# snf4j/snf4j

Measured on AMD Instinct MI355X. Metric: WebSocket frame decode GiB/s device-resident at 1/2/4/8 MI355X; % HBM peak, higher is better.
Workload: dtype u8; 1 GPU; 1048576 x 4096 B masked TEXT frames per GPU, 1024 sessions per GPU, unmask + UTF-8 validation, server-side decode (FrameDecoder+FrameUtf8Validator); frames_per_gpu=1048576, payload_bytes=4096, wire_bytes_per_gpu=4303355904, sessions_per_gpu=1024, parallelism=sessions sharded over 1 GPU(s), one process per GPU, no data-path collective

## Files before the change

snf4j_amd/csrc/api.hip:

```cpp
#include <stdarg.h>
#include <stdio.h>
#include <stdlib.h>
#include <string.h>

#include <algorithm>
#include <atomic>
#include <string>
#include <vector>

#include "wsgpu_internal.h"

using namespace ws;

namespace {

std::atomic<uint64_t> g_ctx_allocs{0};

const char* const kKernelNames[K_COUNT] = {"k_parse",   "k_scan",     "k_link",     "k_piecesN",
                                           "k_final",    "k_enc_len",  "k_enc_scan",
                                           "k_enc_piecesN", "k_enc_final", "k_enc_desc", "k_agg_plan", "k_agg_gather", "k_inflate", "k_hs_accept", "k_infl_tok", "k_infl_fast", "k_hs_validate",
                                           "k_defl_plan", "k_defl_prep", "k_defl_match", "k_defl_parse", "k_defl_final", "k_defl_serial",
                                           "k_defl_trees", "k_defl_emit", "k_defl_hist", "k_defl_match_lds", "k_defl_links"};

struct DevBuf {
// ... 16 lines not shown
    p = nullptr;
    n = 0;
  }
};

struct EventPair {
  int kid;
  hipEvent_t a, b;
};

struct HostSlot {
  DevBuf wire, off, sf, state, payload, desc, result;
  hipEvent_t ev_in = nullptr, ev_k = nullptr, ev_state = nullptr, ev_out = nullptr;
  bool used = false;
};

}

struct wsg_ctx {
  int device = 0;
  hipStream_t stream = nullptr;
  bool own_stream = false;
  std::string err;
  DevBuf rec, vflag, slink, edge, blk_sum, blk_max, chunk, sess_err, total, pieces;
  DevBuf esess, elast_close, epieces, epidx;
  DevBuf a_code, a_last, a_pl, a_cl, a_blk, a_sess_err, a_pieces;
  DevBuf v_desc;
  DevBuf i_tok, i_lit, i_stat, i_tab, i_tabcnt, i_fast, i_ord;
  DevBuf i_split;
  DevBuf i_tok2, i_lit2;
  DevBuf d_flags, d_fout, d_fsym, d_ff, d_fs, d_sums, d_S, d_link, d_res, d_tres, d_strips, d_ftail, d_chunks, d_sym, d_tw, d_ssym,
      d_blocks;
  int defl_serial = 0;
  int64_t stage_fail = 0;
  int defl_lds = 1;
  int infl_tokens = 1;
  uint32_t infl_lanes = 262144;
  uint32_t infl_tabs = 32768;
  int infl_fast = 1;
  int infl_lds = 1;
  int infl_order = 1;
  int infl_split = 0;
  int fused_scan = 1;
  int agg_units = 2;
  uint32_t agg_grid = 65536;
  uint32_t agg_fold = 0xFFFFFFFFu;
  uint64_t tok_frames = 0, tok_payload_len = 0;
// ... 118 lines not shown
  wsg_ctx* c = new wsg_ctx();
  c->device = device;
  if (stream) {
    c->stream = (hipStream_t)stream;
  } else {
    if (hipStreamCreateWithFlags(&c->stream, hipStreamNonBlocking) != hipSuccess) {
      delete c;
      return WSG_API_EHIP;
    }
    c->own_stream = true;
  }
  *out = c;
  return WSG_API_OK;
}

int wsg_close(wsg_ctx* c) {
  if (!c) return WSG_API_EINVAL;
  (void)hipSetDevice(c->device);
  if (c->s_in) (void)hipStreamSynchronize(c->s_in);
  (void)hipStreamSynchronize(c->stream);
  if (c->s_out) (void)hipStreamSynchronize(c->s_out);
  drain_timing(c);
  for (auto e : c->free_events) (void)hipEventDestroy(e);
  DevBuf* bufs[] = {&c->rec,     &c->vflag, &c->chunk,    &c->edge,     &c->blk_sum,  &c->blk_max,   &c->sess_err,
                    &c->total,   &c->pieces, &c->slink, &c->esess,   &c->elast_close, &c->epieces, &c->epidx, &c->h_wire, &c->h_off,    &c->h_sf,
                    &c->h_state, &c->h_payload, &c->h_desc, &c->h_result, &c->h_frames, &c->h_closed,
                    &c->h_wire_off};
  for (DevBuf* b : bufs) b->release();
  DevBuf* abufs[] = {&c->a_code, &c->a_last, &c->a_pl, &c->a_cl,
                     &c->a_blk,  &c->a_sess_err, &c->a_pieces, &c->v_desc, &c->i_tok, &c->i_lit,
                     &c->i_stat, &c->i_tab, &c->i_tabcnt, &c->i_fast, &c->i_ord, &c->i_split,
                     &c->i_tok2, &c->i_lit2};
  for (DevBuf* b : abufs) b->release();
  for (HostSlot& hs : c->slot) {
    DevBuf* sb[] = {&hs.wire, &hs.off, &hs.sf, &hs.state, &hs.payload, &hs.desc, &hs.result};
    for (DevBuf* b : sb) b->release();
    hipEvent_t evs[] = {hs.ev_in, hs.ev_k, hs.ev_state, hs.ev_out};
    for (hipEvent_t e : evs)
      if (e) (void)hipEventDestroy(e);
  }
  if (c->s_in) (void)hipStreamDestroy(c->s_in);
  if (c->s_out) (void)hipStreamDestroy(c->s_out);
  if (c->own_stream) (void)hipStreamDestroy(c->stream);
  delete c;
  return WSG_API_OK;
}

// ... 71 lines not shown
  for (int i = 0; i < K_COUNT && i < max_kernels; ++i) {
    if (out_ms) out_ms[i] = c->ms[i];
    if (out_count) out_count[i] = c->count[i];
  }
  return K_COUNT;
}

int wsg_reset_timing(wsg_ctx* c) {
  if (!c) return WSG_API_EINVAL;
  drain_timing(c);
  memset(c->ms, 0, sizeof c->ms);
  memset(c->count, 0, sizeof c->count);
  return WSG_API_OK;
}

static int ensure_decode_ws(wsg_ctx* c, uint64_t n_frames, uint32_t n_sessions, uint64_t wire_len) {
  const uint64_t F = n_frames ? n_frames : 1;
  const uint64_t nblk = (F + DBLOCK - 1) / DBLOCK;
  HIP_TRY(c, c->pieces.ensure((piece_bound(wire_len, F) + 8) * sizeof(PieceDesc)));
  HIP_TRY(c, c->rec.ensure(F * sizeof(FrameRec)));
  HIP_TRY(c, c->vflag.ensure(F));
  HIP_TRY(c, c->slink.ensure(3 * (uint64_t)(n_sessions ? n_sessions : 1) * sizeof(int32_t)));
  HIP_TRY(c, c->edge.ensure(2 * F * sizeof(uint32_t)));
  HIP_TRY(c, c->blk_sum.ensure(nblk * sizeof(uint64_t)));
  HIP_TRY(c, c->blk_max.ensure(4 * ((nblk + 3) & ~3ull) * sizeof(int32_t)));
  HIP_TRY(c, c->chunk.ensure((nblk / SCAN_CHUNK + 1) * (sizeof(uint64_t) + 4 * sizeof(int32_t))));
  HIP_TRY(c, c->sess_err.ensure((uint64_t)(n_sessions ? n_sessions : 1) * sizeof(uint64_t), 0xff, c->stream));
  HIP_TRY(c, c->total.ensure(sizeof(uint64_t)));
  return WSG_API_OK;
}

static int ensure_encode_ws(wsg_ctx* c, uint64_t n_frames) {
  const uint64_t F = n_frames ? n_frames : 1;
  const uint64_t nblk = (F + BLOCK - 1) / BLOCK;
  HIP_TRY(c, c->esess.ensure(F * sizeof(uint32_t)));
  HIP_TRY(c, c->elast_close.ensure(F * sizeof(int32_t)));
  HIP_TRY(c, c->blk_sum.ensure(nblk * sizeof(uint64_t)));
  HIP_TRY(c, c->blk_max.ensure(3 * nblk * sizeof(int32_t)));
  return WSG_API_OK;
}

static constexpr uint64_t INFL_RESIDENT_LANES = 65536;
static bool infl_pairs(const wsg_ctx* c, uint64_t n_frames) {
  return c->infl_lds && (c->infl_split == 2 || (c->infl_split == 1 && 2 * n_frames <= INFL_RESIDENT_LANES));
}
static uint64_t infl_lane_count(const wsg_ctx* c, uint64_t n_frames) {
// ... 87 lines not shown
    return set_err(c, WSG_API_ERANGE, "payload_cap below wsg_decode_payload_bound()");
  HIP_TRY(c, hipSetDevice(c->device));
  int rc = ensure_decode_ws(c, n_frames, n_sessions, wire_len);
  if (rc) return rc;
  DecodeArgs a;
  a.wire = wire;
  a.wire_len = wire_len;
  a.frame_off = frame_off;
  a.n_frames = n_frames;
  a.session_first = session_first;
  a.n_sessions = n_sessions;
  a.client_mode = cfg->client_mode != 0;
  a.allow_ext = cfg->allow_extensions != 0;
  a.validate = cfg->validate_utf8 != 0;
  a.max_payload = cfg->max_payload_len;
  a.state = state;
  a.payload_out = payload_out;
  a.desc = desc_out;
  a.result = result_out;
  a.rec = (FrameRec*)c->rec.p;
  a.vflag = (uint8_t*)c->vflag.p;
  a.slink = (int32_t*)c->slink.p;
  a.edge = (uint32_t*)c->edge.p;
  a.blk_sum = (uint64_t*)c->blk_sum.p;
  a.blk_max = (int32_t*)c->blk_max.p;
  a.chunk_sum = (uint64_t*)c->chunk.p;
  a.chunk_max = (int32_t*)(a.chunk_sum + (n_frames + DBLOCK - 1) / DBLOCK / SCAN_CHUNK + 1);
  a.sess_err = (uint64_t*)c->sess_err.p;
  a.total = (uint64_t*)c->total.p;
  a.pieces = (PieceDesc*)c->pieces.p;
  a.nblk = (uint32_t)((n_frames + DBLOCK - 1) / DBLOCK);
  a.n_pieces = piece_bound(wire_len, n_frames);
  a.validator_only = 0;
  a.in_desc = nullptr;
  a.sparse = (cfg->flags & WSG_CFG_SPARSE) != 0;
  a.fused_scan = a.nblk <= FUSED_SCAN_MAX_BLOCKS && c->fused_scan;
  if (n_frames) {
    timed(c, K_PARSE, [&] { launch_parse(a, c->stream); });
    if (!a.fused_scan) timed(c, K_SCAN, [&] { launch_scan(a, c->stream); });
    timed(c, K_LINK, [&] { launch_link(a, c->stream); });
    timed(c, K_UNMASK, [&] { launch_pieces(a, c->stream, piece_bound(wire_len, n_frames)); });
  }
  timed(c, K_FINAL, [&] { launch_final(a, c->stream); });
  HIP_TRY(c, hipGetLastError());
  return WSG_API_OK;
}
// ... 8 lines not shown
  HIP_TRY(c, hipSetDevice(c->device));
  int rc = ensure_decode_ws(c, n_frames, n_sessions, payload_len);
  if (rc) return rc;
  HIP_TRY(c, c->v_desc.ensure((n_frames + 1) * sizeof(wsg_frame_desc)));
  DecodeArgs a;
  a.wire = payload;
  a.wire_len = payload_len;
  a.frame_off = nullptr;
  a.n_frames = n_frames;
  a.session_first = session_first;
  a.n_sessions = n_sessions;
  a.client_mode = 0;
  a.allow_ext = 1;
  a.validate = 1;
  a.max_payload = INT64_MAX;
  a.state = state;
  a.payload_out = nullptr;
  a.desc = (wsg_frame_desc*)c->v_desc.p;
  a.result = result_out;
  a.rec = (FrameRec*)c->rec.p;
  a.vflag = (uint8_t*)c->vflag.p;
  a.slink = (int32_t*)c->slink.p;
  a.edge = (uint32_t*)c->edge.p;
  a.blk_sum = (uint64_t*)c->blk_sum.p;
  a.blk_max = (int32_t*)c->blk_max.p;
  a.chunk_sum = (uint64_t*)c->chunk.p;
  a.chunk_max = (int32_t*)(a.chunk_sum + (n_frames + DBLOCK - 1) / DBLOCK / SCAN_CHUNK + 1);
  a.sess_err = (uint64_t*)c->sess_err.p;
  a.total = (uint64_t*)c->total.p;
  a.pieces = (PieceDesc*)c->pieces.p;
  a.nblk = (uint32_t)((n_frames + DBLOCK - 1) / DBLOCK);
  a.n_pieces = piece_bound(payload_len, n_frames);
  a.validator_only = 1;
  a.in_desc = desc;
  a.sparse = 0;
  a.fused_scan = a.nblk <= FUSED_SCAN_MAX_BLOCKS && c->fused_scan;
  if (n_frames) {
    timed(c, K_PARSE, [&] { launch_vparse(a, c->stream); });
    if (!a.fused_scan) timed(c, K_SCAN, [&] { launch_scan(a, c->stream); });
    timed(c, K_LINK, [&] { launch_link(a, c->stream); });
    timed(c, K_UNMASK, [&] { launch_vpieces(a, c->stream, a.n_pieces); });
  }
  timed(c, K_FINAL, [&] { launch_final(a, c->stream); });
  HIP_TRY(c, hipGetLastError());
  return WSG_API_OK;
}
// ... 878 lines not shown
```

snf4j_amd/csrc/decode.hip:

```cpp
#include "wsgpu_internal.h"
#include "wsgpu_scan.h"

namespace ws {

__device__ bool utf8_valid_run(const uint8_t* wire, uint64_t off, uint32_t n, uint32_t mask, uint32_t phase0) {
  uint32_t p1 = 0, p2 = 0, p3 = 0;
  for (uint32_t i = 0; i < n; ++i) {
    uint32_t b = wire[off + i] ^ ((mask >> (8 * ((phase0 + i) & 3))) & 0xffu);
    if (utf8_err_byte(p3, p2, p1, b)) return false;
    p3 = p2; p2 = p1; p1 = b;
  }
  return !utf8_incomplete(p3, p2, p1);
}

struct DAgg {
  uint64_t sum;
  int32_t m0, m1, m2;
  uint32_t c3;
};
constexpr DAgg DAGG_ID = {0ull, -1, -1, -1, 0u};
constexpr uint32_t C3_RESET = 1u << 26;
constexpr uint32_t C3_PENDING = 1u << 27;

__device__ __forceinline__ uint32_t carry_op(uint32_t x, uint32_t y) {
  if (y & C3_RESET) return y;
  const uint32_t nx = (x >> 24) & 3u, ny = (y >> 24) & 3u;
  const uint32_t n = nx + ny < 3u ? nx + ny : 3u;
  return ((x & 0xffffffu) >> (8 * ny)) | (y & 0xffffffu) | (n << 24) | (x & (C3_RESET | C3_PENDING));
}
__device__ __forceinline__ DAgg agg_op(const DAgg& x, const DAgg& y) {
  DAgg r;
  r.sum = x.sum + y.sum;
  r.m0 = x.m0 > y.m0 ? x.m0 : y.m0;
  r.m1 = x.m1 > y.m1 ? x.m1 : y.m1;
  r.m2 = x.m2 > y.m2 ? x.m2 : y.m2;
  r.c3 = carry_op(x.c3, y.c3);
  return r;
}
template <int CTRL, int RM>
__device__ __forceinline__ DAgg agg_dpp(const DAgg& v) {
  DAgg t;
  t.sum = dpp_u64<CTRL, RM>(v.sum, 0ull);
  t.m0 = (int32_t)dpp_u32<CTRL, RM>((uint32_t)v.m0, 0xffffffffu);
  t.m1 = (int32_t)dpp_u32<CTRL, RM>((uint32_t)v.m1, 0xffffffffu);
  t.m2 = (int32_t)dpp_u32<CTRL, RM>((uint32_t)v.m2, 0xffffffffu);
  t.c3 = dpp_u32<CTRL, RM>(v.c3, 0u);
  return t;
}

__device__ __forceinline__ uint32_t tail_c3(const wsg_session_state& st) {
  const uint32_t n = st.tail_len < 3 ? st.tail_len : 3u;
  const uint32_t t = (uint32_t)st.tail[0] | ((uint32_t)st.tail[1] << 8) | ((uint32_t)st.tail[2] << 16);
  return C3_RESET | (n << 24) | ((t << (24 - 8 * n)) & 0xffffffu);
}

__device__ __forceinline__ uint32_t resolve_c3(uint32_t c, const wsg_session_state& st) {
  return (c & C3_PENDING) ? carry_op(tail_c3(st), c & ~(C3_RESET | C3_PENDING)) : c;
}

__device__ __forceinline__ DAgg frame_agg(uint64_t k, const FrameRec& r, uint32_t l3, bool sess_first) {
  DAgg v;
// ... 172 lines not shown
}

__global__ __launch_bounds__(DBLOCK) void k_parse(DecodeArgs a) {
  const uint64_t k = (uint64_t)blockIdx.x * DBLOCK + threadIdx.x;
  DAgg v = DAGG_ID;
  if (k < a.n_frames) {
    const uint64_t o = a.frame_off[k], e = a.sparse ? a.wire_len : a.frame_off[k + 1];
    uint32_t d[6];
    const uint64_t a4 = o & ~3ull;
    if (a4 + 24 <= a.wire_len) {
      const uint32_t* p = (const uint32_t*)(a.wire + a4);
#pragma unroll
      for (int j = 0; j < 6; ++j) d[j] = p[j];
    } else {
#pragma unroll
      for (int j = 0; j < 6; ++j) d[j] = 0u;
#pragma unroll
      for (uint32_t b = 0; b < 24u; ++b)
        if (a4 + b < a.wire_len) d[b >> 2] |= (uint32_t)a.wire[a4 + b] << (8 * (b & 3));
    }
    v = parse_one(a, k, o, e, d, wave_session(a, k));
  }
  DAgg tot;
  block_excl_scan_t(v, &tot, DAGG_ID);
  if (threadIdx.x == 0) store_blk(a, blockIdx.x, tot);
}

__device__ __forceinline__ uint32_t plain_byte(const DecodeArgs& a, uint64_t i) { return i < a.wire_len ? a.wire[i] : 0u; }
__device__ __forceinline__ uint32_t plain_word(const DecodeArgs& a, uint64_t i) {
  const uint64_t q = i & ~3ull;
  if (q + 8 <= a.wire_len) {
    const uint32_t lo = *(const uint32_t*)(a.wire + q), hi = *(const uint32_t*)(a.wire + q + 4);
    return alignbyte(hi, lo, (uint32_t)(i & 3u));
  }
  return plain_byte(a, i) | (plain_byte(a, i + 1) << 8) | (plain_byte(a, i + 2) << 16) | (plain_byte(a, i + 3) << 24);
}

__global__ __launch_bounds__(DBLOCK) void k_vparse(DecodeArgs a) {
  const uint64_t k = (uint64_t)blockIdx.x * DBLOCK + threadIdx.x;
  VAgg v = VAGG_ID;
  if (k < a.n_frames) {
    const uint32_t s = wave_session(a, k);
    const wsg_frame_desc d = a.in_desc[k];
    const uint32_t op = d.opcode & 15u, fin = (d.flags >> 7) & 1u, rsv = (d.flags >> 4) & 7u;
    const uint32_t len = d.payload_len;
    const uint64_t src = d.payload_off;
    uint32_t l3 = 0;
    if (op <= WSG_OP_TEXT && len && !fin) {
      const uint32_t nf = len < 3 ? len : 3;
      const uint32_t keep = nf >= 3 ? 0xffffffu : (nf == 2 ? 0xffffu : 0xffu);
      l3 = (plain_word(a, src + len - nf) & keep) << (8 * (3 - nf));
    }
    a.edge[a.n_frames + k] = l3;
    FrameRec r;
    r.src = src;
    r.len = len;
    r.mask = 0;
    r.code = (fin ? CODE_FIN : 0u) | (rsv << CODE_RSV_SHIFT) | (op << CODE_OP_SHIFT);
    r.sess = s;
    a.rec[k] = r;
    const bool first = k == a.session_first[s];
    v = vframe_agg(r, l3, first, first ? &a.state[s] : nullptr);
  }
  VAgg tot;
  block_excl_scan_t(v, &tot, VAGG_ID);
  if (threadIdx.x == 0) store_blk(a, blockIdx.x, tot);
}

__device__ __forceinline__ void store_chunk(const DecodeArgs& a, uint32_t c, const DAgg& t) {
  a.chunk_sum[c] = t.sum;
  a.chunk_max[4 * c + 0] = t.m0;
  a.chunk_max[4 * c + 1] = t.m1;
  a.chunk_max[4 * c + 2] = t.m2;
  a.chunk_max[4 * c + 3] = (int32_t)t.c3;
}
__device__ __forceinline__ void store_chunk(const DecodeArgs& a, uint32_t c, const VAgg& t) {
  a.chunk_sum[c] = t.sum;
  a.chunk_max[4 * c + 0] = (int32_t)t.fa;
  a.chunk_max[4 * c + 1] = (int32_t)t.fb;
}
__device__ __forceinline__ void load_chunk(const DecodeArgs& a, uint32_t c, DAgg& e) {
  e.sum = a.chunk_sum[c];
  e.m0 = a.chunk_max[4 * c + 0];
  e.m1 = a.chunk_max[4 * c + 1];
  e.m2 = a.chunk_max[4 * c + 2];
  e.c3 = (uint32_t)a.chunk_max[4 * c + 3];
}
__device__ __forceinline__ void load_chunk(const DecodeArgs& a, uint32_t c, VAgg& e) {
// ... 24 lines not shown
    ex = agg_op(ex, e[i]);
  }
  if (threadIdx.x == 0) store_chunk(a, blockIdx.x, tot);
}

__device__ bool seam_utf8_error(uint32_t c3, uint32_t f3, uint32_t len, bool fin) {
  const uint32_t nc = (c3 >> 24) & 3u, nh = len < 3 ? len : 3u, n = nc + nh;
  const uint64_t win = (uint64_t)((c3 & 0xffffffu) >> (24 - 8 * nc)) | ((uint64_t)f3 << (8 * nc));
  for (uint32_t i = nc; i < n; ++i) {
    const uint32_t p1 = i >= 1 ? (uint32_t)(win >> (8 * (i - 1))) & 0xffu : 0u;
    const uint32_t p2 = i >= 2 ? (uint32_t)(win >> (8 * (i - 2))) & 0xffu : 0u;
    const uint32_t p3 = i >= 3 ? (uint32_t)(win >> (8 * (i - 3))) & 0xffu : 0u;
    if (utf8_err_byte(p3, p2, p1, (uint32_t)(win >> (8 * i)) & 0xffu)) return true;
  }
  if (fin && len < 3) {
    const uint32_t t1 = n >= 1 ? (uint32_t)(win >> (8 * (n - 1))) & 0xffu : 0u;
    const uint32_t t2 = n >= 2 ? (uint32_t)(win >> (8 * (n - 2))) & 0xffu : 0u;
    const uint32_t t3 = n >= 3 ? (uint32_t)(win >> (8 * (n - 3))) & 0xffu : 0u;
    if (utf8_incomplete(t3, t2, t1)) return true;
  }
  return false;
}

__device__ __forceinline__ void write_pieces(const DecodeArgs& a, bool live, uint64_t k, const FrameRec& r,
                                             uint64_t ex_sum, bool validate, bool cont, int lane) {
  const uint64_t slot = live ? (uint64_t)((r.len + 15u) & ~15u) : 0ull;
  const uint64_t slot_end = ex_sum + slot;
  const uint32_t pc0 = (uint32_t)((ex_sum + PIECE - 1) / PIECE);
  const uint32_t cnt = slot ? (uint32_t)((slot_end + PIECE - 1) / PIECE) - pc0 : 0u;
  uint32_t cum = cnt;
  cum = wave_incl_sum_u32(cum);
  const uint32_t T = (uint32_t)__builtin_amdgcn_readlane((int)cum, 63);
  cum -= cnt;
  if (!T) return;
  const uint32_t fk = (uint32_t)k | (validate ? 0x80000000u : 0u) | ((live && (r.code & CODE_FIN)) ? 0x40000000u : 0u);
  for (uint32_t t = lane; t < ((T + 63u) & ~63u); t += 64) {
    int o = 0;
#pragma unroll
    for (int step = 32; step >= 1; step >>= 1)
      if ((uint32_t)__shfl((int)cum, o + step, 64) <= t) o += step;
    const uint32_t o_cum = (uint32_t)__shfl((int)cum, o, 64);
    const uint32_t o_pc0 = (uint32_t)__shfl((int)pc0, o, 64);
    const uint64_t o_out = ((uint64_t)(uint32_t)__shfl((int)(uint32_t)(ex_sum >> 32), o, 64) << 32) |
                           (uint32_t)__shfl((int)(uint32_t)ex_sum, o, 64);
    const uint64_t o_src = ((uint64_t)(uint32_t)__shfl((int)(uint32_t)(r.src >> 32), o, 64) << 32) |
                           (uint32_t)__shfl((int)(uint32_t)r.src, o, 64);
    const uint32_t o_len = (uint32_t)__shfl((int)r.len, o, 64);
    const uint32_t o_mask = (uint32_t)__shfl((int)r.mask, o, 64);
    const uint32_t o_fk = (uint32_t)__shfl((int)fk, o, 64);
    const bool o_cont = __shfl((int)cont, o, 64) != 0;
    if (t >= T) continue;
    const uint64_t pc = (uint64_t)o_pc0 + (t - o_cum);
    if (pc >= a.n_pieces) continue;
    const uint64_t ps = pc * PIECE;
    const uint64_t o_end = o_out + ((o_len + 15u) & ~15u);
    const uint32_t j0 = (uint32_t)(ps - o_out);
    const uint32_t left = o_len - j0;
    const bool single = o_end >= ps + PIECE || (uint64_t)(o_fk & 0x3fffffffu) + 1 == a.n_frames;
// ... 25 lines not shown
        t.sum += s0.x + s0.y + s1.x + s1.y;
        t.m0 = max(max(t.m0, max(x0.x, x0.y)), max(x0.z, x0.w));
        t.m1 = max(max(t.m1, max(x1.x, x1.y)), max(x1.z, x1.w));
        t.m2 = max(max(t.m2, max(x2.x, x2.y)), max(x2.z, x2.w));
        c3s[b] = (uint32_t)x3.x;
        c3s[b + 1] = (uint32_t)x3.y;
        c3s[b + 2] = (uint32_t)x3.z;
        c3s[b + 3] = (uint32_t)x3.w;
      } else {
        for (uint32_t i = b; i < nb; ++i) {
          const DAgg e = load_blk(a, i);
          t.sum += e.sum;
          t.m0 = t.m0 > e.m0 ? t.m0 : e.m0;
          t.m1 = t.m1 > e.m1 ? t.m1 : e.m1;
          t.m2 = t.m2 > e.m2 ? t.m2 : e.m2;
          c3s[i] = e.c3;
        }
      }
    }
    __syncthreads();
    const uint32_t per = (blockIdx.x + DBLOCK - 1) / DBLOCK;
    const uint32_t b0 = threadIdx.x * per, b1 = b0 + per < blockIdx.x ? b0 + per : blockIdx.x;
    for (uint32_t b = b0; b < b1; ++b) t.c3 = carry_op(t.c3, c3s[b]);
    block_excl_scan_t(t, &bp, DAGG_ID);
  } else {
    bp = DAGG_ID;
    for (uint32_t c = 0; c < blockIdx.x / SCAN_CHUNK; ++c) {
      DAgg e;
      e.sum = a.chunk_sum[c];
      e.m0 = a.chunk_max[4 * c + 0];
      e.m1 = a.chunk_max[4 * c + 1];
      e.m2 = a.chunk_max[4 * c + 2];
      e.c3 = (uint32_t)a.chunk_max[4 * c + 3];
      bp = agg_op(bp, e);
    }
    bp = agg_op(bp, load_blk(a, blockIdx.x));
  }
  {
    const uint64_t k = (uint64_t)blockIdx.x * DBLOCK + threadIdx.x;
    const bool live = k < a.n_frames;
    FrameRec r = {0ull, 0u, 0u, 0u, 0u};
    DAgg v = DAGG_ID;
    wsg_session_state st = {};
    bool first = false;
    if (live) {
      r = a.rec[k];
      const uint32_t l3 = (code_is_data(r.code) && r.len && !(r.code & CODE_FIN)) ? a.edge[a.n_frames + k] : 0u;
      first = k == a.session_first[r.sess];
      st = a.state[r.sess];
      v = frame_agg(k, r, l3, first);
    }
    DAgg tot;
    DAgg ex = agg_op(bp, block_excl_scan_t(v, &tot, DAGG_ID));
    if (blockIdx.x + 1 == a.nblk && threadIdx.x == 0) *a.total = bp.sum + tot.sum;
    uint32_t validate = 0;
    if (live) {
      const int32_t jd = ex.m0 >> 1, jm = ex.m1 >> 1;
      const uint32_t s = r.sess;
      const int32_t sf = (int32_t)a.session_first[s];
      const uint32_t op = code_op(r.code);
      uint32_t frag_err = 0;
      bool text = false;
      if (!code_pre(r.code)) {
        const bool frag = jd >= sf ? !(ex.m0 & 1) : (st.fragmentation != 0);
        if (!a.validator_only) frag_err = rules_frag(op, frag);
        if (a.validate) {
          text = op == WSG_OP_TEXT;
          if (op == WSG_OP_CONTINUATION) text = jm >= sf ? (ex.m1 & 1) != 0 : (st.text_open != 0);
        }
      }
      uint32_t status = code_pre(r.code) ? code_pre(r.code) : (frag_err ? frag_err : code_post(r.code));
      if (!status && ex.sum + r.len > a.n_pieces * PIECE) status = WSG_E_BATCH;
      if (!status && text && op == WSG_OP_CONTINUATION &&
          seam_utf8_error(first ? tail_c3(st) : resolve_c3(ex.c3, st), a.edge[k], r.len, (r.code & CODE_FIN) != 0))
        status = WSG_E_TEXT_UTF8;
      validate = (text && !status) ? 1u : 0u;
      a.vflag[k] = (uint8_t)(validate | ((validate && op == WSG_OP_CONTINUATION) ? 2u : 0u));
      wsg_frame_desc d;
      d.payload_off = ex.sum;
      d.payload_len = r.len;
      d.opcode = (uint8_t)op;
      d.flags = (uint8_t)(((r.code & CODE_FIN) ? 0x80u : 0u) | (((r.code >> CODE_RSV_SHIFT) & 7u) << 4) |
                          ((r.code & CODE_MASKED) ? 1u : 0u));
      d.status = (uint16_t)status;
      a.desc[k] = d;
      if (status) atomicMin((unsigned long long*)&a.sess_err[s], (unsigned long long)k);
      if (k + 1 == a.session_first[s + 1]) {
        a.slink[s] = code_is_data(r.code) ? (int32_t)k : jd;
        a.slink[a.n_sessions + s] = code_is_start(r.code) ? (int32_t)k : jm;
        a.slink[2 * a.n_sessions + s] = (int32_t)resolve_c3(first ? v.c3 : carry_op(ex.c3, v.c3), st);
      }
    }
    write_pieces(a, live, k, r, ex.sum, validate != 0, live && code_op(r.code) == WSG_OP_CONTINUATION, lane);
  }
}

__global__ __launch_bounds__(DBLOCK) void k_vlink(DecodeArgs a) {
  const int lane = threadIdx.x & 63;
  VAgg bp;
  if (a.fused_scan) {
    __shared__ uint32_t fas[FUSED_SCAN_MAX_BLOCKS], fbs[FUSED_SCAN_MAX_BLOCKS];
    const uint32_t nb = blockIdx.x, st = blk_stride(a);
    uint64_t sum = 0;
    for (uint32_t b = threadIdx.x; b < nb; b += DBLOCK) {
      sum += a.blk_sum[b];
      fas[b] = (uint32_t)a.blk_max[b];
      fbs[b] = (uint32_t)a.blk_max[st + b];
    }
    __syncthreads();
    const uint32_t per = (nb + DBLOCK - 1) / DBLOCK;
    const uint32_t b0 = threadIdx.x * per, b1 = b0 + per < nb ? b0 + per : nb;
    VAgg t = VAGG_ID;
    for (uint32_t b = b0; b < b1; ++b) t = agg_op(t, VAgg{0ull, fas[b], fbs[b]});
    t.sum = sum;
    block_excl_scan_t(t, &bp, VAGG_ID);
  } else {
    bp = VAGG_ID;
    for (uint32_t c = 0; c < blockIdx.x / SCAN_CHUNK; ++c) {
      VAgg e;
      load_chunk(a, c, e);
      bp = agg_op(bp, e);
    }
    VAgg e;
    load_blk(a, blockIdx.x, e);
    bp = agg_op(bp, e);
  }
  const uint64_t k = (uint64_t)blockIdx.x * DBLOCK + threadIdx.x;
  const bool live = k < a.n_frames;
  FrameRec r = {0ull, 0u, 0u, 0u, 0u};
  VAgg v = VAGG_ID;
  wsg_session_state st = {};
  bool first = false;
  if (live) {
    r = a.rec[k];
    const uint32_t l3 = (r.len && !(r.code & CODE_FIN)) ? a.edge[a.n_frames + k] : 0u;
    first = k == a.session_first[r.sess];
    if (first) st = a.state[r.sess];
    v = vframe_agg(r, l3, first, &st);
  }
  VAgg tot;
  const VAgg ex = agg_op(bp, block_excl_scan_t(v, &tot, VAGG_ID));
  if (blockIdx.x + 1 == a.nblk && threadIdx.x == 0) *a.total = bp.sum + tot.sum;
  bool validate = false, seam = false;
  if (live) {
    const uint32_t s = r.sess;
    const uint32_t op = code_op(r.code);
    const bool open = first ? st.text_open != 0 : vopen(ex.fa) != 0;
    const uint32_t carry = first ? (st.text_open ? tail_c3(st) & VC_MASK : 0u) : ex.fb;
    validate = op == WSG_OP_TEXT || (op == WSG_OP_CONTINUATION && open);
    seam = validate && open;
    uint32_t status = 0;
    if (ex.sum + r.len > a.n_pieces * PIECE) status = WSG_E_BATCH;
    if (!status && seam) {
      const uint32_t nh = r.len < 3 ? r.len : 3u;
      const uint32_t f3 = nh ? plain_word(a, r.src) & (0xffffffu >> (8 * (3 - nh))) : 0u;
      if (seam_utf8_error(carry, f3, r.len, (r.code & CODE_FIN) != 0)) status = WSG_E_TEXT_UTF8;
    }
    validate = validate && !status;
    seam = seam && validate;
    a.vflag[k] = (uint8_t)((validate ? 1u : 0u) | (seam ? 2u : 0u));
    wsg_frame_desc d;
    d.payload_off = ex.sum;
    d.payload_len = r.len;
    d.opcode = (uint8_t)op;
    d.flags = (uint8_t)(((r.code & CODE_FIN) ? 0x80u : 0u) | (((r.code >> CODE_RSV_SHIFT) & 7u) << 4));
// ... 492 lines not shown
```

snf4j_amd/csrc/wsgpu_internal.h:

```cpp
#pragma once
#include <stdint.h>

#include <hip/hip_runtime.h>

#include "ws_rules.h"

namespace ws {

struct FrameRec {
  uint64_t src;
  uint32_t len;
  uint32_t mask;
  uint32_t code;
  uint32_t sess;
};

constexpr uint32_t CODE_PRE_SHIFT = 0;
constexpr uint32_t CODE_POST_SHIFT = 5;
constexpr uint32_t CODE_FRAG_SHIFT = 10;
constexpr uint32_t CODE_FIN = 1u << 16;
constexpr uint32_t CODE_RSV_SHIFT = 17;
constexpr uint32_t CODE_MASKED = 1u << 20;
constexpr uint32_t CODE_OP_SHIFT = 24;

__host__ __device__ inline uint32_t code_pre(uint32_t c) { return (c >> CODE_PRE_SHIFT) & 31u; }
__host__ __device__ inline uint32_t code_post(uint32_t c) { return (c >> CODE_POST_SHIFT) & 31u; }
__host__ __device__ inline uint32_t code_frag(uint32_t c) { return (c >> CODE_FRAG_SHIFT) & 31u; }
__host__ __device__ inline uint32_t code_op(uint32_t c) { return (c >> CODE_OP_SHIFT) & 15u; }
__host__ __device__ inline bool code_is_data(uint32_t c) { return code_op(c) <= 2u && !code_pre(c); }
__host__ __device__ inline bool code_is_start(uint32_t c) {
  return (code_op(c) == 1u || code_op(c) == 2u) && !code_pre(c);
}

constexpr int BLOCK = 256;
#ifndef WSG_AGG_BLOCK
#define WSG_AGG_BLOCK 512
#endif
constexpr int ABLOCK = WSG_AGG_BLOCK;
#ifndef WSG_DBLOCK
#define WSG_DBLOCK 256
#endif
constexpr int DBLOCK = WSG_DBLOCK;
constexpr uint32_t PIECE = 1024;
constexpr int PIECES_PER_WAVE = 2;
#ifndef WSG_VPIECES
#define WSG_VPIECES 4
#endif
constexpr int VPIECES_PER_WAVE = WSG_VPIECES;
#ifndef WSG_ENC_PIECES
#define WSG_ENC_PIECES 2
#endif
constexpr int ENC_PIECES_PER_WAVE = WSG_ENC_PIECES;

__host__ __device__ inline uint64_t piece_bound(uint64_t wire_len, uint64_t n_frames) {
  return (wire_len + 16 * n_frames) / PIECE + 1;
}

struct PieceDesc {
  uint64_t info;
  uint32_t mask;
  uint32_t frame;
};
constexpr uint32_t PDF_INDEX = 0x3fffffffu;
constexpr uint32_t PDF_CONT = 0x80000000u;
constexpr uint64_t PD_SRC_MASK = (1ull << 48) - 1;
constexpr uint32_t PD_NB_SHIFT = 48;
constexpr uint64_t PD_VALIDATE = 1ull << 59;
constexpr uint64_t PD_FIRST = 1ull << 60;
constexpr uint64_t PD_MULTI = 1ull << 61;
constexpr uint64_t PD_LAST = 1ull << 62;
constexpr uint64_t PD_FIN = 1ull << 63;

struct DecodeArgs {
  const uint8_t* wire;
  uint64_t wire_len;
  const uint64_t* frame_off;
  uint64_t n_frames;
  const uint32_t* session_first;
  uint32_t n_sessions;
  int32_t client_mode, allow_ext, validate;
  int64_t max_payload;
  int32_t validator_only;
  const wsg_frame_desc* in_desc;
  int32_t sparse;
  wsg_session_state* state;
  uint8_t* payload_out;
  wsg_frame_desc* desc;
  wsg_session_result* result;
  FrameRec* rec;
  uint8_t* vflag;
  int32_t* slink;
  uint32_t* edge;
  uint64_t* blk_sum;
  int32_t* blk_max;
  uint64_t* chunk_sum;
  int32_t* chunk_max;
  uint64_t* sess_err;
  uint64_t* total;
  struct PieceDesc* pieces;
  uint64_t n_pieces;
  uint32_t nblk;
  int32_t fused_scan;
};

constexpr uint32_t FUSED_SCAN_MAX_BLOCKS = 4096;
constexpr uint32_t SCAN_CHUNK = 4096;

struct EncodeArgs {
  int32_t client_mode;
  const uint8_t* payload;
  uint64_t payload_len;
  const wsg_encode_frame* frames;
  uint64_t n_frames;
  const uint32_t* session_first;
  uint32_t n_sessions;
// ... 151 lines not shown
  uint64_t* sums;
  uint8_t* S;
  uint16_t* link;
  uint32_t* res;
  uint32_t* tres;
  uint8_t* strips;
  uint8_t* ftail;
  uint64_t* chunks;
  uint64_t chunk_cap;
  uint32_t* sym;
  DeflBlock* blocks;
  void* tw;
  uint32_t n_lanes;
  uint32_t* ssym;
};

enum KernelId {
  K_PARSE = 0, K_SCAN, K_LINK, K_UNMASK, K_FINAL,
  K_ENC_LEN, K_ENC_SCAN, K_ENC_EMIT, K_ENC_FINAL, K_ENC_DESC, K_AGG, K_AGG_GATHER, K_INFLATE, K_HS_ACCEPT, K_INFL_TOK, K_INFL_FAST, K_HS_VALIDATE,
  K_DEFL_PLAN, K_DEFL_PREP, K_DEFL_MATCH, K_DEFL_PARSE, K_DEFL_FINAL, K_DEFL_SERIAL, K_DEFL_TREES, K_DEFL_EMIT,
  K_DEFL_HIST, K_DEFL_MATCH_LDS, K_DEFL_LINKS, K_COUNT
};

hipError_t ctx_wait_prev_state(wsg_ctx* c);
hipError_t ctx_record_out(wsg_ctx* c, hipEvent_t e);
hipStream_t ctx_stream(wsg_ctx* c);
hipStream_t ctx_out_stream(wsg_ctx* c);
void ctx_copy_tuning(wsg_ctx* dst, const wsg_ctx* src);
int ctx_device(wsg_ctx* c);
bool ctx_inflate_two_phase(const wsg_ctx* c);
uint8_t* ctx_async_payload(wsg_ctx* c);
bool ctx_stage_fail(wsg_ctx* c);
uint64_t ctx_alloc_count();
int ctx_reserve_stages(wsg_ctx* c, uint64_t max_frames, uint32_t max_sessions, uint64_t payload_len,
                       uint64_t agg_cap);
int inflate_tok_phase(wsg_ctx* tokc, const wsg_frame_desc* desc, uint64_t n_frames, const uint32_t* session_first,
                      uint32_t n_sessions, const uint8_t* payload, uint64_t payload_len);
int inflate_replay_phase(wsg_ctx* c, wsg_ctx* tokc, const uint32_t* tmap, int no_context, const wsg_frame_desc* desc,
                         uint64_t n_frames, const uint32_t* session_first, uint32_t n_sessions, const uint8_t* payload,
                         uint64_t payload_len, wsg_inflate_state* state, uint8_t* window, uint8_t* out,
                         const uint64_t* out_off, wsg_frame_desc* out_desc, wsg_session_result* out_result,
                         uint32_t* replay_from);

void launch_parse(const DecodeArgs& a, hipStream_t s);
void launch_scan(const DecodeArgs& a, hipStream_t s);
void launch_link(const DecodeArgs& a, hipStream_t s);
// ... 30 lines not shown
                   wsg_deflate_state* state, uint8_t* session_mem, uint8_t* out, uint64_t out_cap,
                   wsg_frame_desc* out_desc, const DeflBounds* bounds, uint64_t* out_total);

void launch_defl_plan(const DeflArgs& a, hipStream_t s);
void launch_defl_prep(const DeflArgs& a, hipStream_t s);
void launch_defl_match(const DeflArgs& a, hipStream_t s);
void launch_defl_match_lds(const DeflArgs& a, hipStream_t s);
void launch_defl_links(const DeflArgs& a, hipStream_t s);
void launch_defl_parse(const DeflArgs& a, hipStream_t s);
void launch_defl_hist(const DeflArgs& a, hipStream_t s, uint64_t n_blocks);
void launch_defl_trees(const DeflArgs& a, hipStream_t s, uint64_t n_blocks);
void launch_defl_emit(const DeflArgs& a, hipStream_t s);
void launch_defl_final(const DeflArgs& a, hipStream_t s);
void launch_defl_serial(const DeflArgs& a, hipStream_t s);
size_t defl_treework_bytes();
constexpr uint64_t zd_lit_bufsize() { return 16384; }
constexpr uint64_t zd_strip() { return 260; }

void launch_hs_accept(const wsg_hs_config& cfg, const uint8_t* req, const uint64_t* req_off, uint32_t n,
                      uint8_t* resp, wsg_hs_result* result, hipStream_t s);
void launch_hs_validate(const wsg_hs_config& cfg, const uint8_t* resp, const uint64_t* resp_off, const uint8_t* keys,
                        uint32_t n, uint8_t* expected, wsg_hs_result* result, hipStream_t s);
__host__ __device__ int hs_frame_len(const uint8_t* d, int64_t len, int* capped, int64_t* lines_end);


}
```

snf4j_amd/csrc/wsgpu_scan.h:

```cpp
#pragma once
#include "wsgpu_internal.h"

namespace ws {

typedef unsigned int u32x4 __attribute__((ext_vector_type(4)));

__device__ __forceinline__ uint64_t shfl_up_u64(uint64_t v, int d) {
  uint32_t lo = __shfl_up((unsigned)v, d, 64), hi = __shfl_up((unsigned)(v >> 32), d, 64);
  return ((uint64_t)hi << 32) | lo;
}

struct Agg {
  uint64_t sum;
  int32_t m0, m1, m2;
};

__device__ __forceinline__ Agg agg_op(const Agg& x, const Agg& y) {
  Agg r;
  r.sum = x.sum + y.sum;
  r.m0 = x.m0 > y.m0 ? x.m0 : y.m0;
  r.m1 = x.m1 > y.m1 ? x.m1 : y.m1;
  r.m2 = x.m2 > y.m2 ? x.m2 : y.m2;
  return r;
}
// ... 42 lines not shown
  v = agg_op(agg_dpp<DPP_ROW_BCAST31, 0xc>(v), v);
  return v;
}

template <class T>
__device__ inline T block_excl_scan_t(T v, T* total, const T id) {
  __shared__ T wsum[16];
  const int lane = threadIdx.x & 63, wid = threadIdx.x >> 6, nw = blockDim.x >> 6;
  T inc = wave_incl_scan(v);
  if (lane == 63) wsum[wid] = inc;
  __syncthreads();
  T pre = id, tot = id;
  for (int i = 0; i < nw; ++i) {
    if (i < wid) pre = agg_op(pre, wsum[i]);
    tot = agg_op(tot, wsum[i]);
  }
  __syncthreads();
  T ex = agg_dpp<DPP_WAVE_SHR1, 0xf>(inc);
  if (lane == 0) ex = id;
  *total = tot;
  return agg_op(pre, ex);
}

__device__ inline Agg block_excl_scan(Agg v, Agg* total) { return block_excl_scan_t(v, total, AGG_ID); }

__device__ __forceinline__ uint32_t find_session_in(const uint32_t* sf, uint32_t lo, uint32_t hi, uint64_t k) {
  while (lo < hi) {
    uint32_t mid = (lo + hi + 1) >> 1;
    if ((uint64_t)sf[mid] <= k) lo = mid;
    else hi = mid - 1;
  }
  return lo;
}
__device__ __forceinline__ uint32_t find_session(const uint32_t* sf, uint32_t n_sessions, uint64_t k) {
  uint32_t lo = 0, hi = n_sessions ? n_sessions - 1 : 0;
  while (lo < hi) {
    uint32_t mid = (lo + hi + 1) >> 1;
    if ((uint64_t)sf[mid] <= k) lo = mid;
    else hi = mid - 1;
  }
  return lo;
}

__device__ __forceinline__ uint32_t wave_find_session(const uint32_t* sf, uint32_t n_sessions, uint64_t n_frames,
                                                      uint64_t k) {
  const uint32_t kw = __builtin_amdgcn_readfirstlane((uint32_t)(k & ~63ull));
// ... 14 lines not shown
```

Baseline: 2822 GiB/s.

## Persist block-local exclusive prefixes from parse and reuse them in link

The parse kernel now stores each frame's block-local exclusive scan result (sum, packed max indices, carry) into a new FramePre buffer. The link kernel reads it instead of recomputing frame_agg and a second block-wide scan, and only recomputes frame_agg at session ends. The block-prefix combine switches from a full exclusive scan to a cheaper block reduction. Separately, write_pieces gains a direct per-lane path when every lane has at most a few pieces, which skips the wave-cooperative expansion. The cost is an extra 16-byte-per-frame write and read, plus header changes so the aggregate types can be shared with host code.

```diff
diff --git a/snf4j_amd/csrc/api.hip b/snf4j_amd/csrc/api.hip
--- a/snf4j_amd/csrc/api.hip
+++ b/snf4j_amd/csrc/api.hip
@@ -62,7 +62,7 @@
   hipStream_t stream = nullptr;
   bool own_stream = false;
   std::string err;
-  DevBuf rec, vflag, slink, edge, blk_sum, blk_max, chunk, sess_err, total, pieces;
+  DevBuf rec, vflag, slink, edge, pre, blk_sum, blk_max, chunk, sess_err, total, pieces;
   DevBuf esess, elast_close, epieces, epidx;
   DevBuf a_code, a_last, a_pl, a_cl, a_blk, a_sess_err, a_pieces;
   DevBuf v_desc;
@@ -227,7 +227,7 @@
   if (c->s_out) (void)hipStreamSynchronize(c->s_out);
   drain_timing(c);
   for (auto e : c->free_events) (void)hipEventDestroy(e);
-  DevBuf* bufs[] = {&c->rec,     &c->vflag, &c->chunk,    &c->edge,     &c->blk_sum,  &c->blk_max,   &c->sess_err,
+  DevBuf* bufs[] = {&c->rec,     &c->vflag, &c->chunk,    &c->edge,     &c->pre,      &c->blk_sum,  &c->blk_max,   &c->sess_err,
                     &c->total,   &c->pieces, &c->slink, &c->esess,   &c->elast_close, &c->epieces, &c->epidx, &c->h_wire, &c->h_off,    &c->h_sf,
                     &c->h_state, &c->h_payload, &c->h_desc, &c->h_result, &c->h_frames, &c->h_closed,
                     &c->h_wire_off};
@@ -345,6 +345,7 @@
   HIP_TRY(c, c->vflag.ensure(F));
   HIP_TRY(c, c->slink.ensure(3 * (uint64_t)(n_sessions ? n_sessions : 1) * sizeof(int32_t)));
   HIP_TRY(c, c->edge.ensure(2 * F * sizeof(uint32_t)));
+  HIP_TRY(c, c->pre.ensure(F * sizeof(FramePre)));
   HIP_TRY(c, c->blk_sum.ensure(nblk * sizeof(uint64_t)));
   HIP_TRY(c, c->blk_max.ensure(4 * ((nblk + 3) & ~3ull) * sizeof(int32_t)));
   HIP_TRY(c, c->chunk.ensure((nblk / SCAN_CHUNK + 1) * (sizeof(uint64_t) + 4 * sizeof(int32_t))));
@@ -478,6 +479,7 @@
   a.vflag = (uint8_t*)c->vflag.p;
   a.slink = (int32_t*)c->slink.p;
   a.edge = (uint32_t*)c->edge.p;
+  a.pre = (FramePre*)c->pre.p;
   a.blk_sum = (uint64_t*)c->blk_sum.p;
   a.blk_max = (int32_t*)c->blk_max.p;
   a.chunk_sum = (uint64_t*)c->chunk.p;
@@ -532,6 +534,7 @@
   a.vflag = (uint8_t*)c->vflag.p;
   a.slink = (int32_t*)c->slink.p;
   a.edge = (uint32_t*)c->edge.p;
+  a.pre = (FramePre*)c->pre.p;
   a.blk_sum = (uint64_t*)c->blk_sum.p;
   a.blk_max = (int32_t*)c->blk_max.p;
   a.chunk_sum = (uint64_t*)c->chunk.p;
diff --git a/snf4j_amd/csrc/decode.hip b/snf4j_amd/csrc/decode.hip
--- a/snf4j_amd/csrc/decode.hip
+++ b/snf4j_amd/csrc/decode.hip
@@ -1,5 +1,9 @@
 #include "wsgpu_internal.h"
 #include "wsgpu_scan.h"
+
+#ifndef WSG_PIECE_DIRECT_MAX
+#define WSG_PIECE_DIRECT_MAX 8
+#endif
 
 namespace ws {
 
@@ -13,30 +17,8 @@
   return !utf8_incomplete(p3, p2, p1);
 }
 
-struct DAgg {
-  uint64_t sum;
-  int32_t m0, m1, m2;
-  uint32_t c3;
-};
 constexpr DAgg DAGG_ID = {0ull, -1, -1, -1, 0u};
-constexpr uint32_t C3_RESET = 1u << 26;
-constexpr uint32_t C3_PENDING = 1u << 27;
-
-__device__ __forceinline__ uint32_t carry_op(uint32_t x, uint32_t y) {
-  if (y & C3_RESET) return y;
-  const uint32_t nx = (x >> 24) & 3u, ny = (y >> 24) & 3u;
-  const uint32_t n = nx + ny < 3u ? nx + ny : 3u;
-  return ((x & 0xffffffu) >> (8 * ny)) | (y & 0xffffffu) | (n << 24) | (x & (C3_RESET | C3_PENDING));
-}
-__device__ __forceinline__ DAgg agg_op(const DAgg& x, const DAgg& y) {
-  DAgg r;
-  r.sum = x.sum + y.sum;
-  r.m0 = x.m0 > y.m0 ? x.m0 : y.m0;
-  r.m1 = x.m1 > y.m1 ? x.m1 : y.m1;
-  r.m2 = x.m2 > y.m2 ? x.m2 : y.m2;
-  r.c3 = carry_op(x.c3, y.c3);
-  return r;
-}
+
 template <int CTRL, int RM>
 __device__ __forceinline__ DAgg agg_dpp(const DAgg& v) {
   DAgg t;
@@ -255,7 +237,8 @@
     v = parse_one(a, k, o, e, d, wave_session(a, k));
   }
   DAgg tot;
-  block_excl_scan_t(v, &tot, DAGG_ID);
+  const DAgg ex = block_excl_scan_t(v, &tot, DAGG_ID);
+  if (k < a.n_frames) a.pre[k] = pre_pack(ex, blockIdx.x * DBLOCK);
   if (threadIdx.x == 0) store_blk(a, blockIdx.x, tot);
 }
 
@@ -296,7 +279,8 @@
     v = vframe_agg(r, l3, first, first ? &a.state[s] : nullptr);
   }
   VAgg tot;
-  block_excl_scan_t(v, &tot, VAGG_ID);
+  const VAgg ex = block_excl_scan_t(v, &tot, VAGG_ID);
+  if (k < a.n_frames) a.pre[k] = FramePre{ex.sum, ex.fa, ex.fb};
   if (threadIdx.x == 0) store_blk(a, blockIdx.x, tot);
 }
 
@@ -367,18 +351,37 @@
   return false;
 }
 
+constexpr uint32_t PIECE_DIRECT_MAX = WSG_PIECE_DIRECT_MAX;
 __device__ __forceinline__ void write_pieces(const DecodeArgs& a, bool live, uint64_t k, const FrameRec& r,
                                              uint64_t ex_sum, bool validate, bool cont, int lane) {
   const uint64_t slot = live ? (uint64_t)((r.len + 15u) & ~15u) : 0ull;
   const uint64_t slot_end = ex_sum + slot;
   const uint32_t pc0 = (uint32_t)((ex_sum + PIECE - 1) / PIECE);
   const uint32_t cnt = slot ? (uint32_t)((slot_end + PIECE - 1) / PIECE) - pc0 : 0u;
+  const uint32_t fk = (uint32_t)k | (validate ? 0x80000000u : 0u) | ((live && (r.code & CODE_FIN)) ? 0x40000000u : 0u);
+  if (PIECE_DIRECT_MAX && !__any(cnt > PIECE_DIRECT_MAX)) {
+    for (uint32_t i = 0; i < cnt; ++i) {
+      const uint64_t pc = (uint64_t)pc0 + i;
+      if (pc >= a.n_pieces) break;
+      const uint64_t ps = pc * PIECE;
+      const uint32_t j0 = (uint32_t)(ps - ex_sum);
+      const uint32_t left = r.len - j0;
+      const bool single = slot_end >= ps + PIECE || k + 1 == a.n_frames;
+      PieceDesc d;
+      d.info = ((r.src + j0) & PD_SRC_MASK) | ((uint64_t)(left < PIECE ? left : PIECE) << PD_NB_SHIFT) |
+               (validate ? PD_VALIDATE : 0ull) | (j0 == 0 ? PD_FIRST : 0ull) | (single ? 0ull : PD_MULTI) |
+               (left <= PIECE ? PD_LAST : 0ull) | ((fk & 0x40000000u) ? PD_FIN : 0ull);
+      d.mask = r.mask;
+      d.frame = (fk & PDF_INDEX) | (cont ? PDF_CONT : 0u);
+      a.pieces[pc] = d;
+    }
+    return;
+  }
   uint32_t cum = cnt;
   cum = wave_incl_sum_u32(cum);
   const uint32_t T = (uint32_t)__builtin_amdgcn_readlane((int)cum, 63);
   cum -= cnt;
   if (!T) return;
-  const uint32_t fk = (uint32_t)k | (validate ? 0x80000000u : 0u) | ((live && (r.code & CODE_FIN)) ? 0x40000000u : 0u);
   for (uint32_t t = lane; t < ((T + 63u) & ~63u); t += 64) {
     int o = 0;
 #pragma unroll
@@ -450,7 +453,7 @@
     const uint32_t per = (blockIdx.x + DBLOCK - 1) / DBLOCK;
     const uint32_t b0 = threadIdx.x * per, b1 = b0 + per < blockIdx.x ? b0 + per : blockIdx.x;
     for (uint32_t b = b0; b < b1; ++b) t.c3 = carry_op(t.c3, c3s[b]);
-    block_excl_scan_t(t, &bp, DAGG_ID);
+    bp = block_reduce_t(t, DAGG_ID);
   } else {
     bp = DAGG_ID;
     for (uint32_t c = 0; c < blockIdx.x / SCAN_CHUNK; ++c) {
@@ -468,19 +471,15 @@
     const uint64_t k = (uint64_t)blockIdx.x * DBLOCK + threadIdx.x;
     const bool live = k < a.n_frames;
     FrameRec r = {0ull, 0u, 0u, 0u, 0u};
-    DAgg v = DAGG_ID;
     wsg_session_state st = {};
     bool first = false;
     if (live) {
       r = a.rec[k];
-      const uint32_t l3 = (code_is_data(r.code) && r.len && !(r.code & CODE_FIN)) ? a.edge[a.n_frames + k] : 0u;
       first = k == a.session_first[r.sess];
       st = a.state[r.sess];
-      v = frame_agg(k, r, l3, first);
-    }
-    DAgg tot;
-    DAgg ex = agg_op(bp, block_excl_scan_t(v, &tot, DAGG_ID));
-    if (blockIdx.x + 1 == a.nblk && threadIdx.x == 0) *a.total = bp.sum + tot.sum;
+    }
+    const DAgg ex = agg_op(bp, live ? pre_unpack(a.pre[k], blockIdx.x * DBLOCK) : DAGG_ID);
+    if (k + 1 == a.n_frames) *a.total = ex.sum + ((r.len + 15u) & ~15u);
     uint32_t validate = 0;
     if (live) {
       const int32_t jd = ex.m0 >> 1, jm = ex.m1 >> 1;
@@ -516,6 +515,8 @@
       if (k + 1 == a.session_first[s + 1]) {
         a.slink[s] = code_is_data(r.code) ? (int32_t)k : jd;
         a.slink[a.n_sessions + s] = code_is_start(r.code) ? (int32_t)k : jm;
+        const uint32_t l3 = (code_is_data(r.code) && r.len && !(r.code & CODE_FIN)) ? a.edge[a.n_frames + k] : 0u;
+        const DAgg v = frame_agg(k, r, l3, first);
         a.slink[2 * a.n_sessions + s] = (int32_t)resolve_c3(first ? v.c3 : carry_op(ex.c3, v.c3), st);
       }
     }
@@ -541,7 +542,7 @@
     VAgg t = VAGG_ID;
     for (uint32_t b = b0; b < b1; ++b) t = agg_op(t, VAgg{0ull, fas[b], fbs[b]});
     t.sum = sum;
-    block_excl_scan_t(t, &bp, VAGG_ID);
+    bp = block_reduce_t(t, VAGG_ID);
   } else {
     bp = VAGG_ID;
     for (uint32_t c = 0; c < blockIdx.x / SCAN_CHUNK; ++c) {
@@ -566,9 +567,13 @@
     if (first) st = a.state[r.sess];
     v = vframe_agg(r, l3, first, &st);
   }
-  VAgg tot;
-  const VAgg ex = agg_op(bp, block_excl_scan_t(v, &tot, VAGG_ID));
-  if (blockIdx.x + 1 == a.nblk && threadIdx.x == 0) *a.total = bp.sum + tot.sum;
+  VAgg lp = VAGG_ID;
+  if (live) {
+    const FramePre p = a.pre[k];
+    lp = VAgg{p.sum, p.m, p.c3};
+  }
+  const VAgg ex = agg_op(bp, lp);
+  if (k + 1 == a.n_frames) *a.total = ex.sum + v.sum;
   bool validate = false, seam = false;
   if (live) {
     const uint32_t s = r.sess;
diff --git a/snf4j_amd/csrc/wsgpu_internal.h b/snf4j_amd/csrc/wsgpu_internal.h
--- a/snf4j_amd/csrc/wsgpu_internal.h
+++ b/snf4j_amd/csrc/wsgpu_internal.h
@@ -1,7 +1,9 @@
 #pragma once
 #include <stdint.h>
 
+#ifdef __HIPCC__
 #include <hip/hip_runtime.h>
+#endif
 
 #include "ws_rules.h"
 
@@ -23,12 +25,12 @@
 constexpr uint32_t CODE_MASKED = 1u << 20;
 constexpr uint32_t CODE_OP_SHIFT = 24;
 
-__host__ __device__ inline uint32_t code_pre(uint32_t c) { return (c >> CODE_PRE_SHIFT) & 31u; }
-__host__ __device__ inline uint32_t code_post(uint32_t c) { return (c >> CODE_POST_SHIFT) & 31u; }
-__host__ __device__ inline uint32_t code_frag(uint32_t c) { return (c >> CODE_FRAG_SHIFT) & 31u; }
-__host__ __device__ inline uint32_t code_op(uint32_t c) { return (c >> CODE_OP_SHIFT) & 15u; }
-__host__ __device__ inline bool code_is_data(uint32_t c) { return code_op(c) <= 2u && !code_pre(c); }
-__host__ __device__ inline bool code_is_start(uint32_t c) {
+WS_HD uint32_t code_pre(uint32_t c) { return (c >> CODE_PRE_SHIFT) & 31u; }
+WS_HD uint32_t code_post(uint32_t c) { return (c >> CODE_POST_SHIFT) & 31u; }
+WS_HD uint32_t code_frag(uint32_t c) { return (c >> CODE_FRAG_SHIFT) & 31u; }
+WS_HD uint32_t code_op(uint32_t c) { return (c >> CODE_OP_SHIFT) & 15u; }
+WS_HD bool code_is_data(uint32_t c) { return code_op(c) <= 2u && !code_pre(c); }
+WS_HD bool code_is_start(uint32_t c) {
   return (code_op(c) == 1u || code_op(c) == 2u) && !code_pre(c);
 }
 
@@ -52,7 +54,7 @@
 #endif
 constexpr int ENC_PIECES_PER_WAVE = WSG_ENC_PIECES;
 
-__host__ __device__ inline uint64_t piece_bound(uint64_t wire_len, uint64_t n_frames) {
+WS_HD uint64_t piece_bound(uint64_t wire_len, uint64_t n_frames) {
   return (wire_len + 16 * n_frames) / PIECE + 1;
 }
 
@@ -70,6 +72,55 @@
 constexpr uint64_t PD_MULTI = 1ull << 61;
 constexpr uint64_t PD_LAST = 1ull << 62;
 constexpr uint64_t PD_FIN = 1ull << 63;
+
+struct DAgg {
+  uint64_t sum;
+  int32_t m0, m1, m2;
+  uint32_t c3;
+};
+constexpr uint32_t C3_RESET = 1u << 26;
+constexpr uint32_t C3_PENDING = 1u << 27;
+
+WS_HD uint32_t carry_op(uint32_t x, uint32_t y) {
+  if (y & C3_RESET) return y;
+  const uint32_t nx = (x >> 24) & 3u, ny = (y >> 24) & 3u;
+  const uint32_t n = nx + ny < 3u ? nx + ny : 3u;
+  return ((x & 0xffffffu) >> (8 * ny)) | (y & 0xffffffu) | (n << 24) | (x & (C3_RESET | C3_PENDING));
+}
+WS_HD DAgg agg_op(const DAgg& x, const DAgg& y) {
+  DAgg r;
+  r.sum = x.sum + y.sum;
+  r.m0 = x.m0 > y.m0 ? x.m0 : y.m0;
+  r.m1 = x.m1 > y.m1 ? x.m1 : y.m1;
+  r.m2 = x.m2 > y.m2 ? x.m2 : y.m2;
+  r.c3 = carry_op(x.c3, y.c3);
+  return r;
+}
+
+struct alignas(16) FramePre {
+  uint64_t sum;
+  uint32_t m, c3;
+};
+static_assert(2 * DBLOCK < 1023, "FramePre.m: a block-local frame index and its bit take 10 bits");
+
+WS_HD uint32_t pre_pack_max(int32_t m, uint32_t k0) { return m < 0 ? 0u : (uint32_t)m - (k0 << 1) + 1u; }
+WS_HD int32_t pre_unpack_max(uint32_t f, uint32_t k0) { return f ? (int32_t)((k0 << 1) + f - 1u) : -1; }
+WS_HD FramePre pre_pack(const DAgg& e, uint32_t k0) {
+  FramePre p;
+  p.sum = e.sum;
+  p.m = pre_pack_max(e.m0, k0) | (pre_pack_max(e.m1, k0) << 10) | (pre_pack_max(e.m2, k0) << 20);
+  p.c3 = e.c3;
+  return p;
+}
+WS_HD DAgg pre_unpack(const FramePre& p, uint32_t k0) {
+  DAgg e;
+  e.sum = p.sum;
+  e.m0 = pre_unpack_max(p.m & 1023u, k0);
+  e.m1 = pre_unpack_max((p.m >> 10) & 1023u, k0);
+  e.m2 = pre_unpack_max((p.m >> 20) & 1023u, k0);
+  e.c3 = p.c3;
+  return e;
+}
 
 struct DecodeArgs {
   const uint8_t* wire;
@@ -91,6 +142,7 @@
   uint8_t* vflag;
   int32_t* slink;
   uint32_t* edge;
+  FramePre* pre;
   uint64_t* blk_sum;
   int32_t* blk_max;
   uint64_t* chunk_sum;
@@ -288,6 +340,8 @@
   K_DEFL_HIST, K_DEFL_MATCH_LDS, K_DEFL_LINKS, K_COUNT
 };
 
+#ifdef __HIPCC__
+
 hipError_t ctx_wait_prev_state(wsg_ctx* c);
 hipError_t ctx_record_out(wsg_ctx* c, hipEvent_t e);
 hipStream_t ctx_stream(wsg_ctx* c);
@@ -364,6 +418,6 @@
 void launch_hs_validate(const wsg_hs_config& cfg, const uint8_t* resp, const uint64_t* resp_off, const uint8_t* keys,
                         uint32_t n, uint8_t* expected, wsg_hs_result* result, hipStream_t s);
 __host__ __device__ int hs_frame_len(const uint8_t* d, int64_t len, int* capped, int64_t* lines_end);
-
-
-}
+#endif
+
+}
diff --git a/snf4j_amd/csrc/wsgpu_scan.h b/snf4j_amd/csrc/wsgpu_scan.h
--- a/snf4j_amd/csrc/wsgpu_scan.h
+++ b/snf4j_amd/csrc/wsgpu_scan.h
@@ -88,6 +88,18 @@
   return agg_op(pre, ex);
 }
 
+template <class T>
+__device__ inline T block_reduce_t(T v, const T id) {
+  __shared__ T wtot[16];
+  const int lane = threadIdx.x & 63, wid = threadIdx.x >> 6, nw = blockDim.x >> 6;
+  const T inc = wave_incl_scan(v);
+  if (lane == 63) wtot[wid] = inc;
+  __syncthreads();
+  T tot = id;
+  for (int i = 0; i < nw; ++i) tot = agg_op(tot, wtot[i]);
+  return tot;
+}
+
 __device__ inline Agg block_excl_scan(Agg v, Agg* total) { return block_excl_scan_t(v, total, AGG_ID); }
 
 __device__ __forceinline__ uint32_t find_session_in(const uint32_t* sf, uint32_t lo, uint32_t hi, uint64_t k) {
```

Measured after the change: 2800 GiB/s. About the same (-0.8%).
